# COMP6248-Reproducability-Challenge/selfsupervised-denoising

Hardware: AMD Instinct MI355X
Metric: training patches/sec (64x64 gauss25 SSDN) (higher is better)
Workload: dtype f16

## Files before the change

selfsupervised-denoising_amd/csrc/conv_thin.hip:

```cpp
#include "common.h"
#include <cstring>

#define CT_THREADS 256

template <int MT, bool PACK>
__global__ __launch_bounds__(CT_THREADS) void k_conv_thin(ssdn_conv_args a, int padT, int padB, int padL, int padR, unsigned long long tapmap, int dy0,
                                                          ssdn_pack_input_args pk) {
    extern __shared__ __attribute__((aligned(16))) char smem[];
    const int tid = threadIdx.x, lane = tid & 63, l31 = lane & 31, kh = lane >> 5;
    const int wave = __builtin_amdgcn_readfirstlane(tid >> 6);
    const int tiles_x = a.W >> 6, bands = a.H >> 4;
    int bid = blockIdx.x;
    const int x0 = (bid % tiles_x) << 6; bid /= tiles_x;
    const int y0 = (bid % bands) << 4;
    const int n = bid / bands;
    const int HH = 16 + padT + padB, HW = 64 + padL + padR;
    const h16* wp = (const h16*)a.w;
    half8 af[MT][3];
    f32x16 binit[MT];
#pragma unroll
    for (int mt = 0; mt < MT; ++mt) {
#pragma unroll
        for (int r = 0; r < 3; ++r)
#pragma unroll
            for (int j = 0; j < 8; ++j) {
                const int d = kh * 2 + (j >> 2), c = j & 3;
                const int t = (int)((tapmap >> (4 * (3 * r + (d < 3 ? d : 0)))) & 15u);
                af[mt][r][j] = (d < 3 && c < a.kreal) ? wp[((long long)t * a.Mpad + mt * 32 + l31) * a.Ktot + c] : (h16)0.f;
            }
#pragma unroll
        for (int r = 0; r < 16; ++r) {
            const int m = mt * 32 + (r >> 2) * 8 + kh * 4 + (r & 3);
            binit[mt][r] = m < a.M ? a.bias[m] : 0.f;
        }
    }
    const h16* src = (const h16*)a.src0.p + a.src0.co;
    constexpr int NIT = 6;
    float f32v[NIT][3];
    u32x2_t raw[NIT];
    bool ok[NIT];
#pragma unroll
    for (int it = 0; it < NIT; ++it) {
        const int e = tid + it * CT_THREADS;
        const int hy = e / HW, hx = e - hy * HW;
        const int y = y0 - padT + hy, x = x0 - padL + hx;
        ok[it] = e < HH * HW && (unsigned)y < (unsigned)a.H && (unsigned)x < (unsigned)a.W;
        const int yc = ok[it] ? y : 0, xc = ok[it] ? x : 0;
        if constexpr (PACK) {
            const int r = n / pk.B, b = n - r * pk.B, H = a.H, W = a.W;
            int sy, sx;
            switch (r) {
                case 0: sy = yc; sx = xc; break;
                case 1: sy = xc; sx = W - 1 - yc; break;
                case 2: sy = H - 1 - yc; sx = W - 1 - xc; break;
                default: sy = H - 1 - xc; sx = yc; break;
            }
#pragma unroll
            for (int c = 0; c < 3; ++c) f32v[it][c] = pk.src[(((long long)b * pk.C + (c < pk.C ? c : 0)) * H + sy) * W + sx];
        } else {
            raw[it] = *reinterpret_cast<const u32x2_t*>(src + ((long long)(n * a.H + yc) * a.W + xc) * a.src0.cs);
        }
    }
#pragma unroll
    for (int it = 0; it < NIT; ++it) {
        const int e = tid + it * CT_THREADS;
        u32x2_t v = {0u, 0u};
        if (ok[it]) {
            if constexpr (PACK) {
                h16 c4[3];
#pragma unroll
                for (int c = 0; c < 3; ++c) c4[c] = c < pk.C ? (h16)f32v[it][c] : (h16)0.f;
                v[0] = (unsigned)__builtin_bit_cast(unsigned short, c4[0]) | ((unsigned)__builtin_bit_cast(unsigned short, c4[1]) << 16);
                v[1] = (unsigned)__builtin_bit_cast(unsigned short, c4[2]);
            } else v = raw[it];
        }
        if (e < HH * HW + 1) *reinterpret_cast<u32x2_t*>(smem + e * 8) = v;
    }
    __syncthreads();
    if constexpr (PACK) {
        const int ppx = pk.cpad >> 3;
        for (int e = tid; e < 16 * 64 * ppx; e += CT_THREADS) {
            const int p = e / ppx, piece = e - p * ppx;
            const int ty = p >> 6, tx = p & 63;
            u32x4_t o = {0u, 0u, 0u, 0u};
            if (piece == 0) {
                const u32x2_t v = *reinterpret_cast<const u32x2_t*>(smem + (((ty + padT) * HW + tx + padL) << 3));
                o[0] = v[0]; o[1] = v[1];
            }
            *reinterpret_cast<u32x4_t*>((h16*)pk.dst.p + ((long long)(n * a.H + y0 + ty) * a.W + x0 + tx) * pk.dst.cs + pk.dst.co + piece * 8) = o;
        }
    }
    constexpr int OSTR = MT * 64 + 16;
    char* reg = smem + (((HH * HW + 1) * 8 + 15) & ~15) + wave * (32 * OSTR);
    const int npc = a.M >> 3;
    const unsigned npc_magic = npc <= 1 ? 0u : (unsigned)((0x100000000ull + npc - 1) / npc);
    h16* dst = (h16*)a.dst.p + a.dst.co;
    const int zoff = HH * HW * 8;
#pragma unroll 2
    for (int i = 0; i < 8; ++i) {
        const int q = (wave * 8 + i) * 32 + l31;
        const int ty = q >> 6, tx = q & 63;
        const int pb = (((ty + padT + dy0) * HW + tx + padL - 1) << 3) + kh * 16;
        half8 bf[3];
#pragma unroll
        for (int r = 0; r < 3; ++r) {
            const u32x2_t lo = *reinterpret_cast<const u32x2_t*>(smem + pb + r * HW * 8);
            const u32x2_t hi = *reinterpret_cast<const u32x2_t*>(smem + (kh ? zoff : pb + r * HW * 8 + 8));
            const u32x4_t w4 = {lo[0], lo[1], hi[0], hi[1]};
            bf[r] = __builtin_bit_cast(half8, w4);
        }
        f32x16 acc[MT];
#pragma unroll
        for (int mt = 0; mt < MT; ++mt) {
            acc[mt] = binit[mt];
#pragma unroll
            for (int r = 0; r < 3; ++r) acc[mt] = __builtin_amdgcn_mfma_f32_32x32x16_f16(af[mt][r], bf[r], acc[mt], 0, 0, 0);
        }
#pragma unroll
        for (int mt = 0; mt < MT; ++mt)
#pragma unroll
            for (int g = 0; g < 4; ++g) {
                float v[4];
#pragma unroll
                for (int j = 0; j < 4; ++j) v[j] = acc[mt][g * 4 + j];
#pragma unroll
                for (int j = 0; j < 4; j += 2) {
                    const f32x2_t t = f32x2_t{v[j], v[j + 1]} * LRELU_SLOPE;
                    asm("v_max_f32 %0, %1, %2" : "=v"(v[j]) : "v"(v[j]), "v"(t[0]));
                    asm("v_max_f32 %0, %1, %2" : "=v"(v[j + 1]) : "v"(v[j + 1]), "v"(t[1]));
                }
                u32x2_t o;
                o[0] = pack_f16x2(v[0], v[1]);
                o[1] = pack_f16x2(v[2], v[3]);
                *reinterpret_cast<u32x2_t*>(reg + (i & 1) * (4 * 32 * OSTR) + l31 * OSTR + (mt * 32 + g * 8 + kh * 4) * 2) = o;
            }
        asm volatile("s_waitcnt lgkmcnt(0)" ::: "memory");
        __builtin_amdgcn_wave_barrier();
        const long long pix0 = (long long)(n * a.H + y0 + (((wave * 8 + i) * 32) >> 6)) * a.W + x0 + (((wave * 8 + i) * 32) & 63);
        for (int e = lane; e < 32 * npc; e += 64) {
            const int p = npc_magic ? (int)__umulhi((unsigned)e, npc_magic) : e, cc = e - p * npc;
            const u32x4_t o = *reinterpret_cast<const u32x4_t*>(reg + (i & 1) * (4 * 32 * OSTR) + p * OSTR + cc * 16);
            *reinterpret_cast<u32x4_t*>(dst + (pix0 + p) * a.dst.cs + cc * 8) = o;
            if (a.sign_out) {
                unsigned rq[4];
#pragma unroll
                for (int q = 0; q < 4; ++q) {
                    unsigned t0;
                    asm("v_pk_max_i16 %0, %1, 0" : "=v"(t0) : "v"(o[q]));
                    asm("v_pk_min_i16 %0, %1, %2" : "=v"(rq[q]) : "v"(t0), "s"(0x00010001u));
                }
                const unsigned t01 = (rq[1] << 2) | rq[0], t23 = (rq[3] << 2) | rq[2];
                const unsigned t = (t23 << 4) | t01;
                const unsigned sb = t | (t >> 15);
                ((unsigned char*)a.sign_out)[(pix0 + p) * npc + cc] = (unsigned char)sb;
            }
        }
    }
}

static void thin_pads(const ssdn_conv_args* a, int* padT, int* padB, int* padL, int* padR) {
    int mny = 0, mxy = 0, mnx = 0, mxx = 0;
    for (int t = 0; t < a->ntaps; ++t) {
        mny = a->dy[t] < mny ? a->dy[t] : mny; mxy = a->dy[t] > mxy ? a->dy[t] : mxy;
        mnx = a->dx[t] < mnx ? a->dx[t] : mnx; mxx = a->dx[t] > mxx ? a->dx[t] : mxx;
    }
    *padT = -mny; *padB = mxy; *padL = -mnx; *padR = mxx;
}

static bool thin_window(const ssdn_conv_args* a, unsigned long long* tapmap, int* dy0) {
    int mny = 1 << 30;
    for (int t = 0; t < 9; ++t) mny = a->dy[t] < mny ? a->dy[t] : mny;
    unsigned long long map = 0;
    unsigned seen = 0;
    for (int t = 0; t < 9; ++t) {
        const int r = a->dy[t] - mny, d = a->dx[t] + 1;
        if (r < 0 || r > 2 || d < 0 || d > 2) return false;
        map |= (unsigned long long)t << (4 * (3 * r + d));
        seen |= 1u << (3 * r + d);
    }
    if (seen != 0x1ffu) return false;
    *tapmap = map; *dy0 = mny;
    return true;
}

bool conv_thin_eligible(const ssdn_conv_args* a) {
    if (a->bf16 || a->ntaps != 9 || a->c1 || a->up0 || a->Ktot != 16 || a->c0 != 16 || a->kreal < 1 || a->kreal > 3) return false;
    if (!a->dst.p || a->dst32 || !a->act || !a->bias || a->pool.p || a->mask.p || a->add.p || a->upsum.p || a->unrot.p) return false;
    if ((a->H & 15) || (a->W & 63) || a->M < 8 || (a->M & 7) || a->Mpad > 64 || a->Mpad < 32) return false;
    if (a->src0.cs < 4 || (a->src0.cs & 3) || (a->src0.co & 3)) return false;
    unsigned long long map; int dy0;
    int pt, pb, pl, pr;
    thin_pads(a, &pt, &pb, &pl, &pr);
    if ((16 + pt + pb) * (64 + pl + pr) + 1 > 6 * CT_THREADS) return false;
    return thin_window(a, &map, &dy0);
}

bool conv_thin_fuses_pack(const ssdn_pack_input_args* pk, const ssdn_conv_args* a) {
    if (!conv_thin_eligible(a) || !pk->src || !pk->dst.p) return false;
    if (pk->dst.p != a->src0.p || pk->dst.cs != a->src0.cs || pk->dst.co != a->src0.co) return false;
    if (pk->R * pk->B != a->N || pk->H != a->H || pk->W != a->W || pk->C != a->kreal || pk->C > 3) return false;
    if ((pk->R != 1 && pk->R != 4) || (pk->R == 4 && pk->H != pk->W)) return false;
    return (pk->cpad & 7) == 0 && pk->cpad >= 8 && (pk->dst.cs & 7) == 0 && (pk->dst.co & 7) == 0;
}

int launch_conv_thin(const ssdn_conv_args* a, const ssdn_pack_input_args* pk, hipStream_t s) {
    int pt, pb, pl, pr, dy0 = 0;
    unsigned long long map = 0;
    thin_pads(a, &pt, &pb, &pl, &pr);
    if (!thin_window(a, &map, &dy0)) return ssdn_set_error("conv thin: the taps are not a 3x3 window");
    if (pk && !conv_thin_fuses_pack(pk, a)) return ssdn_set_error("conv thin: this SSDN_OP_PACK_INPUT cannot be folded into the launch");
    const int mt = a->Mpad / 32;
    const size_t lds = (size_t)((((16 + pt + pb) * (64 + pl + pr) + 1) * 8 + 15) & ~15) + 2u * 4u * 32u * (mt * 64 + 16);
    const int grid = a->N * (a->H >> 4) * (a->W >> 6);
    ssdn_pack_input_args none;
    memset(&none, 0, sizeof(none));
    if (pk) {
        if (mt == 2) hipLaunchKernelGGL((k_conv_thin<2, true>), dim3(grid), dim3(CT_THREADS), lds, s, *a, pt, pb, pl, pr, map, dy0, *pk);
        else hipLaunchKernelGGL((k_conv_thin<1, true>), dim3(grid), dim3(CT_THREADS), lds, s, *a, pt, pb, pl, pr, map, dy0, *pk);
    } else {
        if (mt == 2) hipLaunchKernelGGL((k_conv_thin<2, false>), dim3(grid), dim3(CT_THREADS), lds, s, *a, pt, pb, pl, pr, map, dy0, none);
        else hipLaunchKernelGGL((k_conv_thin<1, false>), dim3(grid), dim3(CT_THREADS), lds, s, *a, pt, pb, pl, pr, map, dy0, none);
    }
    SSDN_CHECK_HIP(hipGetLastError());
    return 0;
}
```

Measured before the change: 20680.

## Make thin conv persistent with prefetched halo and LDS-staged weights

Turns the thin 3x3 conv kernel into a persistent grid sized to twice the CU count. Each block loops over tiles and prefetches the next tile's halo into registers while it computes the current one. Weights and bias are loaded once per block through LDS instead of scattered per-lane global reads. Divisions are replaced by host-computed magic multipliers, store offsets are precomputed, and rotated pack inputs are read column-wise for coalescing. The costs are more registers, extra LDS, and an added barrier per tile, and grid sizing now depends on the CU count.

```diff
diff --git a/selfsupervised-denoising_amd/csrc/conv_thin.hip b/selfsupervised-denoising_amd/csrc/conv_thin.hip
--- a/selfsupervised-denoising_amd/csrc/conv_thin.hip
+++ b/selfsupervised-denoising_amd/csrc/conv_thin.hip
@@ -1,160 +1,222 @@
 #include "common.h"
+#include <cstdint>
 #include <cstring>
 
 #define CT_THREADS 256
+
+struct CtMagic { unsigned hw, hh, npc, ppx; };
+static __device__ __forceinline__ int ct_div(int e, unsigned magic) { return magic ? (int)__umulhi((unsigned)e, magic) : e; }
 
 template <int MT, bool PACK>
 __global__ __launch_bounds__(CT_THREADS) void k_conv_thin(ssdn_conv_args a, int padT, int padB, int padL, int padR, unsigned long long tapmap, int dy0,
-                                                          ssdn_pack_input_args pk) {
+                                                          ssdn_pack_input_args pk, int nblocks, CtMagic mg) {
     extern __shared__ __attribute__((aligned(16))) char smem[];
     const int tid = threadIdx.x, lane = tid & 63, l31 = lane & 31, kh = lane >> 5;
     const int wave = __builtin_amdgcn_readfirstlane(tid >> 6);
     const int tiles_x = a.W >> 6, bands = a.H >> 4;
-    int bid = blockIdx.x;
-    const int x0 = (bid % tiles_x) << 6; bid /= tiles_x;
-    const int y0 = (bid % bands) << 4;
-    const int n = bid / bands;
     const int HH = 16 + padT + padB, HW = 64 + padL + padR;
-    const h16* wp = (const h16*)a.w;
-    half8 af[MT][3];
-    f32x16 binit[MT];
-#pragma unroll
-    for (int mt = 0; mt < MT; ++mt) {
-#pragma unroll
-        for (int r = 0; r < 3; ++r)
-#pragma unroll
-            for (int j = 0; j < 8; ++j) {
-                const int d = kh * 2 + (j >> 2), c = j & 3;
-                const int t = (int)((tapmap >> (4 * (3 * r + (d < 3 ? d : 0)))) & 15u);
-                af[mt][r][j] = (d < 3 && c < a.kreal) ? wp[((long long)t * a.Mpad + mt * 32 + l31) * a.Ktot + c] : (h16)0.f;
-            }
-#pragma unroll
-        for (int r = 0; r < 16; ++r) {
-            const int m = mt * 32 + (r >> 2) * 8 + kh * 4 + (r & 3);
-            binit[mt][r] = m < a.M ? a.bias[m] : 0.f;
-        }
-    }
+    constexpr int OSTR = MT * 64 + 16;
+    constexpr int MROWS = MT * 32;
+    char* const obase = smem + (((HH * HW + 1) * 8 + 15) & ~15);
+    char* const wlds = obase + 2 * 4 * 32 * OSTR;
+    char* const blds = wlds + 9 * MROWS * 8;
     const h16* src = (const h16*)a.src0.p + a.src0.co;
     constexpr int NIT = 6;
     float f32v[NIT][3];
     u32x2_t raw[NIT];
     bool ok[NIT];
-#pragma unroll
-    for (int it = 0; it < NIT; ++it) {
-        const int e = tid + it * CT_THREADS;
-        const int hy = e / HW, hx = e - hy * HW;
-        const int y = y0 - padT + hy, x = x0 - padL + hx;
-        ok[it] = e < HH * HW && (unsigned)y < (unsigned)a.H && (unsigned)x < (unsigned)a.W;
-        const int yc = ok[it] ? y : 0, xc = ok[it] ? x : 0;
-        if constexpr (PACK) {
-            const int r = n / pk.B, b = n - r * pk.B, H = a.H, W = a.W;
-            int sy, sx;
-            switch (r) {
-                case 0: sy = yc; sx = xc; break;
-                case 1: sy = xc; sx = W - 1 - yc; break;
-                case 2: sy = H - 1 - yc; sx = W - 1 - xc; break;
-                default: sy = H - 1 - xc; sx = yc; break;
-            }
-#pragma unroll
-            for (int c = 0; c < 3; ++c) f32v[it][c] = pk.src[(((long long)b * pk.C + (c < pk.C ? c : 0)) * H + sy) * W + sx];
-        } else {
-            raw[it] = *reinterpret_cast<const u32x2_t*>(src + ((long long)(n * a.H + yc) * a.W + xc) * a.src0.cs);
-        }
-    }
-#pragma unroll
-    for (int it = 0; it < NIT; ++it) {
-        const int e = tid + it * CT_THREADS;
-        u32x2_t v = {0u, 0u};
-        if (ok[it]) {
+    int slot[NIT];
+    int n, y0, x0;
+    auto load_halo = [&](int blk) {
+        x0 = (blk % tiles_x) << 6; blk /= tiles_x;
+        y0 = (blk % bands) << 4;
+        n = blk / bands;
+        const int rot = PACK ? n / pk.B : 0, b = PACK ? n - rot * pk.B : 0;
+        const float* img = PACK ? pk.src + (long long)b * pk.C * a.H * a.W : nullptr;
+        const h16* simg = src + (long long)n * a.H * a.W * a.src0.cs;
+        const bool colwise = PACK && (rot & 1);
+#pragma unroll
+        for (int it = 0; it < NIT; ++it) {
+            const int e = tid + it * CT_THREADS;
+            int hy, hx;
+            if (colwise) { hx = ct_div(e, mg.hh); hy = e - hx * HH; }
+            else { hy = ct_div(e, mg.hw); hx = e - hy * HW; }
+            const int y = y0 - padT + hy, x = x0 - padL + hx;
+            ok[it] = e < HH * HW && (unsigned)y < (unsigned)a.H && (unsigned)x < (unsigned)a.W;
+            slot[it] = e < HH * HW ? hy * HW + hx : (e == HH * HW ? e : -1);
+            const int yc = ok[it] ? y : 0, xc = ok[it] ? x : 0;
             if constexpr (PACK) {
-                h16 c4[3];
-#pragma unroll
-                for (int c = 0; c < 3; ++c) c4[c] = c < pk.C ? (h16)f32v[it][c] : (h16)0.f;
-                v[0] = (unsigned)__builtin_bit_cast(unsigned short, c4[0]) | ((unsigned)__builtin_bit_cast(unsigned short, c4[1]) << 16);
-                v[1] = (unsigned)__builtin_bit_cast(unsigned short, c4[2]);
-            } else v = raw[it];
-        }
-        if (e < HH * HW + 1) *reinterpret_cast<u32x2_t*>(smem + e * 8) = v;
-    }
-    __syncthreads();
-    if constexpr (PACK) {
-        const int ppx = pk.cpad >> 3;
-        for (int e = tid; e < 16 * 64 * ppx; e += CT_THREADS) {
-            const int p = e / ppx, piece = e - p * ppx;
-            const int ty = p >> 6, tx = p & 63;
-            u32x4_t o = {0u, 0u, 0u, 0u};
-            if (piece == 0) {
-                const u32x2_t v = *reinterpret_cast<const u32x2_t*>(smem + (((ty + padT) * HW + tx + padL) << 3));
-                o[0] = v[0]; o[1] = v[1];
-            }
-            *reinterpret_cast<u32x4_t*>((h16*)pk.dst.p + ((long long)(n * a.H + y0 + ty) * a.W + x0 + tx) * pk.dst.cs + pk.dst.co + piece * 8) = o;
-        }
-    }
-    constexpr int OSTR = MT * 64 + 16;
-    char* reg = smem + (((HH * HW + 1) * 8 + 15) & ~15) + wave * (32 * OSTR);
+                const int H = a.H, W = a.W;
+                int sy, sx;
+                switch (rot) {
+                    case 0: sy = yc; sx = xc; break;
+                    case 1: sy = xc; sx = W - 1 - yc; break;
+                    case 2: sy = H - 1 - yc; sx = W - 1 - xc; break;
+                    default: sy = H - 1 - xc; sx = yc; break;
+                }
+#pragma unroll
+                for (int c = 0; c < 3; ++c) f32v[it][c] = img[(unsigned)((c < pk.C ? c : 0) * H * W + sy * W + sx)];
+            } else {
+                raw[it] = *reinterpret_cast<const u32x2_t*>(simg + (unsigned)((yc * a.W + xc) * a.src0.cs));
+            }
+        }
+    };
+    int blk = blockIdx.x;
+    load_halo(blk);
+    {
+        const h16* wp = (const h16*)a.w;
+        constexpr int NW = (9 * MROWS + CT_THREADS - 1) / CT_THREADS;
+        u32x2_t wv[NW];
+#pragma unroll
+        for (int k = 0; k < NW; ++k) {
+            const int idx = tid + k * CT_THREADS, ws = idx / MROWS, m = idx - ws * MROWS;
+            const int t = (int)((tapmap >> (4 * (ws < 9 ? ws : 0))) & 15u);
+            wv[k] = *reinterpret_cast<const u32x2_t*>(wp + ((long long)t * a.Mpad + m) * a.Ktot);
+        }
+        const float bv = tid < a.M ? a.bias[tid < a.M ? tid : 0] : 0.f;
+        const unsigned m0 = a.kreal >= 2 ? 0xffffffffu : 0x0000ffffu, m1 = a.kreal >= 3 ? 0x0000ffffu : 0u;
+#pragma unroll
+        for (int k = 0; k < NW; ++k) {
+            const int idx = tid + k * CT_THREADS;
+            const u32x2_t v = {wv[k][0] & m0, wv[k][1] & m1};
+            if (idx < 9 * MROWS) *reinterpret_cast<u32x2_t*>(wlds + idx * 8) = v;
+        }
+        if (tid < MROWS) *reinterpret_cast<float*>(blds + tid * 4) = bv;
+    }
+    half8 af[MT][3];
+    f32x16 binit[MT];
     const int npc = a.M >> 3;
-    const unsigned npc_magic = npc <= 1 ? 0u : (unsigned)((0x100000000ull + npc - 1) / npc);
+    constexpr int NSI = 2 * MT;
+    int s_lds[NSI];
+    unsigned s_off[NSI];
+#pragma unroll
+    for (int k = 0; k < NSI; ++k) {
+        const int e = lane + 64 * k, p = ct_div(e, mg.npc), cc = e - p * npc;
+        s_lds[k] = p * OSTR + cc * 16;
+        s_off[k] = (unsigned)(p * a.dst.cs + cc * 8) * 2u;
+    }
     h16* dst = (h16*)a.dst.p + a.dst.co;
     const int zoff = HH * HW * 8;
+    char* reg = obase + wave * (32 * OSTR);
+    for (bool first = true;; first = false) {
+#pragma unroll
+        for (int it = 0; it < NIT; ++it) {
+            u32x2_t v = {0u, 0u};
+            if (ok[it]) {
+                if constexpr (PACK) {
+                    h16 c4[3];
+#pragma unroll
+                    for (int c = 0; c < 3; ++c) c4[c] = c < pk.C ? (h16)f32v[it][c] : (h16)0.f;
+                    v[0] = (unsigned)__builtin_bit_cast(unsigned short, c4[0]) | ((unsigned)__builtin_bit_cast(unsigned short, c4[1]) << 16);
+                    v[1] = (unsigned)__builtin_bit_cast(unsigned short, c4[2]);
+                } else v = raw[it];
+            }
+            if (slot[it] >= 0) *reinterpret_cast<u32x2_t*>(smem + slot[it] * 8) = v;
+        }
+        __syncthreads();
+        if (first) {
+#pragma unroll
+            for (int mt = 0; mt < MT; ++mt) {
+#pragma unroll
+                for (int r = 0; r < 3; ++r) {
+                    const u32x2_t lo = *reinterpret_cast<const u32x2_t*>(wlds + ((3 * r + kh * 2) * MROWS + mt * 32 + l31) * 8);
+                    u32x2_t hi = *reinterpret_cast<const u32x2_t*>(wlds + ((3 * r + 1) * MROWS + mt * 32 + l31) * 8);
+                    if (kh) hi = u32x2_t{0u, 0u};
+                    const u32x4_t w4 = {lo[0], lo[1], hi[0], hi[1]};
+                    af[mt][r] = __builtin_bit_cast(half8, w4);
+                }
+#pragma unroll
+                for (int g = 0; g < 4; ++g) {
+                    const f32x4 b4 = *reinterpret_cast<const f32x4*>(blds + (mt * 32 + g * 8 + kh * 4) * 4);
+#pragma unroll
+                    for (int j = 0; j < 4; ++j) binit[mt][g * 4 + j] = b4[j];
+                }
+            }
+        }
+        const int bn = n, by0 = y0, bx0 = x0;
+        const int nblk = blk + (int)gridDim.x;
+        const bool more = nblk < nblocks;
+        if (more) load_halo(nblk);
+        if constexpr (PACK) {
+            const int ppx = pk.cpad >> 3;
+            char* const pdst = reinterpret_cast<char*>((h16*)pk.dst.p + pk.dst.co + ((long long)(bn * a.H + by0) * a.W + bx0) * pk.dst.cs);
+            for (int e = tid; e < 16 * 64 * ppx; e += CT_THREADS) {
+                const int p = ct_div(e, mg.ppx), piece = e - p * ppx;
+                const int ty = p >> 6, tx = p & 63;
+                u32x4_t o = {0u, 0u, 0u, 0u};
+                if (piece == 0) {
+                    const u32x2_t v = *reinterpret_cast<const u32x2_t*>(smem + (((ty + padT) * HW + tx + padL) << 3));
+                    o[0] = v[0]; o[1] = v[1];
+                }
+                *reinterpret_cast<u32x4_t*>(pdst + (unsigned)((ty * a.W + tx) * pk.dst.cs + piece * 8) * 2u) = o;
+            }
+        }
 #pragma unroll 2
-    for (int i = 0; i < 8; ++i) {
-        const int q = (wave * 8 + i) * 32 + l31;
-        const int ty = q >> 6, tx = q & 63;
-        const int pb = (((ty + padT + dy0) * HW + tx + padL - 1) << 3) + kh * 16;
-        half8 bf[3];
-#pragma unroll
-        for (int r = 0; r < 3; ++r) {
-            const u32x2_t lo = *reinterpret_cast<const u32x2_t*>(smem + pb + r * HW * 8);
-            const u32x2_t hi = *reinterpret_cast<const u32x2_t*>(smem + (kh ? zoff : pb + r * HW * 8 + 8));
-            const u32x4_t w4 = {lo[0], lo[1], hi[0], hi[1]};
-            bf[r] = __builtin_bit_cast(half8, w4);
-        }
-        f32x16 acc[MT];
-#pragma unroll
-        for (int mt = 0; mt < MT; ++mt) {
-            acc[mt] = binit[mt];
-#pragma unroll
-            for (int r = 0; r < 3; ++r) acc[mt] = __builtin_amdgcn_mfma_f32_32x32x16_f16(af[mt][r], bf[r], acc[mt], 0, 0, 0);
-        }
-#pragma unroll
-        for (int mt = 0; mt < MT; ++mt)
-#pragma unroll
-            for (int g = 0; g < 4; ++g) {
-                float v[4];
-#pragma unroll
-                for (int j = 0; j < 4; ++j) v[j] = acc[mt][g * 4 + j];
-#pragma unroll
-                for (int j = 0; j < 4; j += 2) {
-                    const f32x2_t t = f32x2_t{v[j], v[j + 1]} * LRELU_SLOPE;
-                    asm("v_max_f32 %0, %1, %2" : "=v"(v[j]) : "v"(v[j]), "v"(t[0]));
-                    asm("v_max_f32 %0, %1, %2" : "=v"(v[j + 1]) : "v"(v[j + 1]), "v"(t[1]));
-                }
-                u32x2_t o;
-                o[0] = pack_f16x2(v[0], v[1]);
-                o[1] = pack_f16x2(v[2], v[3]);
-                *reinterpret_cast<u32x2_t*>(reg + (i & 1) * (4 * 32 * OSTR) + l31 * OSTR + (mt * 32 + g * 8 + kh * 4) * 2) = o;
-            }
-        asm volatile("s_waitcnt lgkmcnt(0)" ::: "memory");
-        __builtin_amdgcn_wave_barrier();
-        const long long pix0 = (long long)(n * a.H + y0 + (((wave * 8 + i) * 32) >> 6)) * a.W + x0 + (((wave * 8 + i) * 32) & 63);
-        for (int e = lane; e < 32 * npc; e += 64) {
-            const int p = npc_magic ? (int)__umulhi((unsigned)e, npc_magic) : e, cc = e - p * npc;
-            const u32x4_t o = *reinterpret_cast<const u32x4_t*>(reg + (i & 1) * (4 * 32 * OSTR) + p * OSTR + cc * 16);
-            *reinterpret_cast<u32x4_t*>(dst + (pix0 + p) * a.dst.cs + cc * 8) = o;
-            if (a.sign_out) {
-                unsigned rq[4];
-#pragma unroll
-                for (int q = 0; q < 4; ++q) {
-                    unsigned t0;
-                    asm("v_pk_max_i16 %0, %1, 0" : "=v"(t0) : "v"(o[q]));
-                    asm("v_pk_min_i16 %0, %1, %2" : "=v"(rq[q]) : "v"(t0), "s"(0x00010001u));
-                }
-                const unsigned t01 = (rq[1] << 2) | rq[0], t23 = (rq[3] << 2) | rq[2];
-                const unsigned t = (t23 << 4) | t01;
-                const unsigned sb = t | (t >> 15);
-                ((unsigned char*)a.sign_out)[(pix0 + p) * npc + cc] = (unsigned char)sb;
-            }
-        }
+        for (int i = 0; i < 8; ++i) {
+            const int q = (wave * 8 + i) * 32 + l31;
+            const int ty = q >> 6, tx = q & 63;
+            const int pb = (((ty + padT + dy0) * HW + tx + padL - 1) << 3) + kh * 16;
+            half8 bf[3];
+#pragma unroll
+            for (int r = 0; r < 3; ++r) {
+                const u32x2_t lo = *reinterpret_cast<const u32x2_t*>(smem + pb + r * HW * 8);
+                const u32x2_t hi = *reinterpret_cast<const u32x2_t*>(smem + (kh ? zoff : pb + r * HW * 8 + 8));
+                const u32x4_t w4 = {lo[0], lo[1], hi[0], hi[1]};
+                bf[r] = __builtin_bit_cast(half8, w4);
+            }
+            f32x16 acc[MT];
+#pragma unroll
+            for (int mt = 0; mt < MT; ++mt) {
+                acc[mt] = binit[mt];
+#pragma unroll
+                for (int r = 0; r < 3; ++r) acc[mt] = __builtin_amdgcn_mfma_f32_32x32x16_f16(af[mt][r], bf[r], acc[mt], 0, 0, 0);
+            }
+#pragma unroll
+            for (int mt = 0; mt < MT; ++mt)
+#pragma unroll
+                for (int g = 0; g < 4; ++g) {
+                    float v[4];
+#pragma unroll
+                    for (int j = 0; j < 4; ++j) v[j] = acc[mt][g * 4 + j];
+#pragma unroll
+                    for (int j = 0; j < 4; j += 2) {
+                        const f32x2_t t = f32x2_t{v[j], v[j + 1]} * LRELU_SLOPE;
+                        asm("v_max_f32 %0, %1, %2" : "=v"(v[j]) : "v"(v[j]), "v"(t[0]));
+                        asm("v_max_f32 %0, %1, %2" : "=v"(v[j + 1]) : "v"(v[j + 1]), "v"(t[1]));
+                    }
+                    u32x2_t o;
+                    o[0] = pack_f16x2(v[0], v[1]);
+                    o[1] = pack_f16x2(v[2], v[3]);
+                    *reinterpret_cast<u32x2_t*>(reg + (i & 1) * (4 * 32 * OSTR) + l31 * OSTR + (mt * 32 + g * 8 + kh * 4) * 2) = o;
+                }
+            asm volatile("s_waitcnt lgkmcnt(0)" ::: "memory");
+            __builtin_amdgcn_wave_barrier();
+            const long long pix0 = (long long)(bn * a.H + by0 + (((wave * 8 + i) * 32) >> 6)) * a.W + bx0 + (((wave * 8 + i) * 32) & 63);
+            char* const tdst = reinterpret_cast<char*>(dst + pix0 * a.dst.cs);
+            unsigned char* const tsign = (unsigned char*)a.sign_out + pix0 * npc;
+#pragma unroll
+            for (int k = 0; k < NSI; ++k) {
+                if (lane + 64 * k >= 32 * npc) break;
+                const u32x4_t o = *reinterpret_cast<const u32x4_t*>(reg + (i & 1) * (4 * 32 * OSTR) + s_lds[k]);
+                *reinterpret_cast<u32x4_t*>(tdst + s_off[k]) = o;
+                if (a.sign_out) {
+                    unsigned rq[4];
+#pragma unroll
+                    for (int q = 0; q < 4; ++q) {
+                        unsigned t0;
+                        asm("v_pk_max_i16 %0, %1, 0" : "=v"(t0) : "v"(o[q]));
+                        asm("v_pk_min_i16 %0, %1, %2" : "=v"(rq[q]) : "v"(t0), "s"(0x00010001u));
+                    }
+                    const unsigned t01 = (rq[1] << 2) | rq[0], t23 = (rq[3] << 2) | rq[2];
+                    const unsigned t = (t23 << 4) | t01;
+                    const unsigned sb = t | (t >> 15);
+                    tsign[lane + 64 * k] = (unsigned char)sb;
+                }
+            }
+        }
+        if (!more) break;
+        blk = nblk;
+        __syncthreads();
     }
 }
 
@@ -188,6 +250,7 @@
     if (!a->dst.p || a->dst32 || !a->act || !a->bias || a->pool.p || a->mask.p || a->add.p || a->upsum.p || a->unrot.p) return false;
     if ((a->H & 15) || (a->W & 63) || a->M < 8 || (a->M & 7) || a->Mpad > 64 || a->Mpad < 32) return false;
     if (a->src0.cs < 4 || (a->src0.cs & 3) || (a->src0.co & 3)) return false;
+    if ((uintptr_t)a->w & 7) return false;
     unsigned long long map; int dy0;
     int pt, pb, pl, pr;
     thin_pads(a, &pt, &pb, &pl, &pr);
@@ -210,16 +273,20 @@
     if (!thin_window(a, &map, &dy0)) return ssdn_set_error("conv thin: the taps are not a 3x3 window");
     if (pk && !conv_thin_fuses_pack(pk, a)) return ssdn_set_error("conv thin: this SSDN_OP_PACK_INPUT cannot be folded into the launch");
     const int mt = a->Mpad / 32;
-    const size_t lds = (size_t)((((16 + pt + pb) * (64 + pl + pr) + 1) * 8 + 15) & ~15) + 2u * 4u * 32u * (mt * 64 + 16);
-    const int grid = a->N * (a->H >> 4) * (a->W >> 6);
+    const size_t lds = (size_t)((((16 + pt + pb) * (64 + pl + pr) + 1) * 8 + 15) & ~15) + 2u * 4u * 32u * (mt * 64 + 16) + 9u * mt * 32u * 8u + mt * 32u * 4u;
+    const int nblocks = a->N * (a->H >> 4) * (a->W >> 6);
+    const int resident = 2 * ssdn_device_cus();
+    const int grid = nblocks >= 2 * resident ? resident : nblocks;
+    auto magic = [](int d) { return d <= 1 ? 0u : (unsigned)((0x100000000ull + d - 1) / d); };
+    const CtMagic mg = {magic(64 + pl + pr), magic(16 + pt + pb), magic(a->M >> 3), magic(pk ? pk->cpad >> 3 : 1)};
     ssdn_pack_input_args none;
     memset(&none, 0, sizeof(none));
     if (pk) {
-        if (mt == 2) hipLaunchKernelGGL((k_conv_thin<2, true>), dim3(grid), dim3(CT_THREADS), lds, s, *a, pt, pb, pl, pr, map, dy0, *pk);
-        else hipLaunchKernelGGL((k_conv_thin<1, true>), dim3(grid), dim3(CT_THREADS), lds, s, *a, pt, pb, pl, pr, map, dy0, *pk);
+        if (mt == 2) hipLaunchKernelGGL((k_conv_thin<2, true>), dim3(grid), dim3(CT_THREADS), lds, s, *a, pt, pb, pl, pr, map, dy0, *pk, nblocks, mg);
+        else hipLaunchKernelGGL((k_conv_thin<1, true>), dim3(grid), dim3(CT_THREADS), lds, s, *a, pt, pb, pl, pr, map, dy0, *pk, nblocks, mg);
     } else {
-        if (mt == 2) hipLaunchKernelGGL((k_conv_thin<2, false>), dim3(grid), dim3(CT_THREADS), lds, s, *a, pt, pb, pl, pr, map, dy0, none);
-        else hipLaunchKernelGGL((k_conv_thin<1, false>), dim3(grid), dim3(CT_THREADS), lds, s, *a, pt, pb, pl, pr, map, dy0, none);
+        if (mt == 2) hipLaunchKernelGGL((k_conv_thin<2, false>), dim3(grid), dim3(CT_THREADS), lds, s, *a, pt, pb, pl, pr, map, dy0, none, nblocks, mg);
+        else hipLaunchKernelGGL((k_conv_thin<1, false>), dim3(grid), dim3(CT_THREADS), lds, s, *a, pt, pb, pl, pr, map, dy0, none, nblocks, mg);
     }
     SSDN_CHECK_HIP(hipGetLastError());
     return 0;
```

New measurement: 20770, median of 6. About the same (+0.4%).
